# qinhy/Open3D-py-extension

Measured on AMD Instinct MI355X. Metric: Mpoints/sec voxel_down_sample+estimate_normals; ICP iters/sec @ N=10M, higher is better.
Workload: dtype f64

## Files before the change

open3d-py-extension_amd/csrc/grid.hip:

```cpp
#include <type_traits>
#include <utility>

#include "grid.hpp"

namespace o3dx {

__global__ void __launch_bounds__(kBlock) k_grid_count(const float* __restrict__ xyz, int64_t n, GridView g,
                                                       int32_t* __restrict__ count, int32_t* __restrict__ cell,
                                                       int32_t* __restrict__ rank) {
  for (int64_t i = (int64_t)blockIdx.x * blockDim.x + threadIdx.x; i < n; i += (int64_t)gridDim.x * blockDim.x) {
    float x = xyz[3 * i], y = xyz[3 * i + 1], z = xyz[3 * i + 2];
    int cx, cy, cz;
    grid_cell(g, x, y, z, cx, cy, cz);
    const int c = cell_index(g, cx, cy, cz);
    cell[i] = c;
    rank[i] = atomicAdd(&count[c], 1);
  }
}

__global__ void __launch_bounds__(kBlock) k_count_nonzero(const int32_t* __restrict__ count, int64_t nc,
                                                          unsigned long long* __restrict__ out) {
  int64_t local = 0;
  for (int64_t c = (int64_t)blockIdx.x * blockDim.x + threadIdx.x; c < nc; c += (int64_t)gridDim.x * blockDim.x)
    local += count[c] != 0;
// ... 1828 lines not shown
                    wy0 + kVB > d.ny - kEdge || wz0 + kVB > d.nz - kEdge;
  float L = 0.f, U = 0.f;
  int ns = 0, nc = 0;
  if (!fb) {
    if (wide)
      fb = !stile_count_list<Stencil245>(txy, tz, qs, SY, SZ, xpos, q, kneed, d.hlo2, d.rw2, hw, lst, lane, kListMax,
                                         dbg, d, &ns, &nc, &L, &U);
    else
      fb = !stile_count_list<Stencil220>(txy, tz, qs, SY, SZ, xpos, q, kneed, d.hlo2, d.rc2, hw, lst, lane, kListMax,
                                         dbg, d, &ns, &nc, &L, &U);
  }
  if (dbg == 2 || dbg == 3) {
    if (ns + nc == 12345 || L == 12345.f) out[0] = 0.f;
    return;
  }
  if (!fb) {
    const bool over = ns + nc > kListMax;
    if (over && d.stats) atomicAdd(&d.stats[5], 1ull);
    fb = over ||
         !stile_finish<KMAX>(
             q, kneed, ns, nc, L, U, lst, lane,
             [&](int p) { return make_float4(txy[p].x, txy[p].y, tz[p], 0.f); }, prior, oi, out, d.nbr,
             [&](int p) {
               const int bz_ = p / kSZ, r = p - bz_ * kSZ, by_ = r / kSY, bx_ = r - by_ * kSY;
               return __float_as_int(
                   d.vox[(gx0 + bx_) + (int64_t)d.nx * ((gy0 + by_) + (int64_t)d.ny * (gz0 + bz_))].w);
             },
             d.kd2, dbg == 4);
  }
  if (fb) {
    if (d.stats) atomicAdd(&d.stats[4], 1ull);
    const int at = atomicAdd(fb_len, 1);
    fb_list[at] = (int32_t)vq;
  }
}

constexpr int kWaveBnd = 64;
constexpr int kWaveRefineAt = 32;
constexpr int kWavesPerBlock = 4;
constexpr int kWaveCache = 512;

__device__ __forceinline__ void wave_sync() {
  __builtin_amdgcn_fence(__ATOMIC_RELEASE, "wavefront");
  __builtin_amdgcn_wave_barrier();
  __builtin_amdgcn_fence(__ATOMIC_ACQUIRE, "wavefront");
}

__device__ __forceinline__ int lanes_below(uint64_t mask) {
  return (int)__builtin_amdgcn_mbcnt_hi((uint32_t)(mask >> 32), __builtin_amdgcn_mbcnt_lo((uint32_t)mask, 0u));
}

constexpr int kWaveMaxS = 5;
constexpr int kWaveRows = 128;

__device__ __forceinline__ int wave_rows(const GridView& g, const float4 q, int cx, int cy, int cz, int S, float r2,
                                         int lane, int32_t* __restrict__ ra, int32_t* __restrict__ rp) {
  const int side = 2 * S + 1, nr = side * side;
  int carry = 0;
  if (lane == 0) rp[0] = 0;
  for (int h = 0; h * 64 < nr; ++h) {
    const int row = lane + 64 * h;
    int a = 0, len = 0;
    if (row < nr) {
      const int z = cz + row / side - S, y = cy + row % side - S;
      if (z >= 0 && z < g.nz && y >= 0 && y < g.ny) {
        const float y0 = g.oy + (float)y * g.h, z0 = g.oz + (float)z * g.h, sl = 2.0f * g.slack;
        const float dy = fmaxf(fmaxf(y0 - q.y, q.y - (y0 + g.h)) - sl, 0.0f);
        const float dz = fmaxf(fmaxf(z0 - q.z, q.z - (z0 + g.h)) - sl, 0.0f);
        const float rem = r2 - fmaf(dy, dy, dz * dz);
        if (rem > 0.0f) {
          const float rx = sqrtf(rem) + sl;
          const int x0 = max(max(cx - S, 0), (int)floorf((q.x - rx - g.ox) * g.inv_h));
          const int x1 = min(min(cx + S, g.nx - 1), (int)floorf((q.x + rx - g.ox) * g.inv_h));
          if (x0 <= x1) {
            const int rb = g.nx * (y + g.ny * z);
            a = cell_start(g, rb + x0);
            len = cell_start(g, rb + x1 + 1) - a;
          }
        }
      }
    }
    const int inc = wave_incl_scan(len) + carry;
    if (row < nr) {
      ra[row] = a;
      rp[row + 1] = inc;
    }
    carry = __shfl(inc, 63, 64);
  }
  wave_sync();
  return carry;
}

#define O3DX_WAVE_SCAN(S, BODY)                                                  \
  {                                                                              \
    int row_ = 0;                                                                \
    for (int b_ = 0; b_ < ncand; b_ += 64 * WU) {                                \
      float4 v_[WU];                                                             \
      int p_[WU];                                                                \
      _Pragma("unroll") for (int u_ = 0; u_ < WU; ++u_) {                        \
        const int f_ = b_ + u_ * 64 + lane;                                      \
        p_[u_] = -1;                                                             \
        if (f_ < ncand) {                                                        \
          while (rp[row_ + 1] <= f_) ++row_;                                     \
          p_[u_] = ra[row_] + (f_ - rp[row_]);                                   \
        }                                                                        \
        v_[u_] = g.pts[p_[u_] >= 0 ? p_[u_] : 0];                                \
      }                                                                          \
      _Pragma("unroll") for (int u_ = 0; u_ < WU; ++u_) {                        \
        const int pp = p_[u_];                                                   \
        const bool valid = pp >= 0;                                              \
        const int fidx = b_ + u_ * 64 + lane;                                    \
        const float d2 = dist2_f32(q, v_[u_].x, v_[u_].y, v_[u_].z);             \
        (void)fidx;                                                              \
        BODY                                                                     \
      }                                                                          \
    }                                                                            \
  }

#define O3DX_WAVE_SCAN_L(BODY)                                                   \
  for (int b_ = 0; b_ < ncand; b_ += 64) {                                       \
    const int f_ = b_ + lane;                                                    \
    const bool valid = f_ < ncand;                                               \
    const float d2 = valid ? cd2[f_] : 0.0f;                                     \
    const int pp = valid ? cpos[f_] : -1;                                        \
    (void)pp;                                                                    \
    BODY                                                                         \
  }
#define O3DX_WAVE_ANY(BODY)        \
  if (cached) {                    \
    O3DX_WAVE_SCAN_L(BODY)         \
  } else {                         \
    O3DX_WAVE_SCAN(S, BODY)        \
  }

struct Deferred {
  double* mom = nullptr;
  int32_t* row = nullptr;
  int64_t cap = 0;
};

__global__ void __launch_bounds__(kBlock) k_finish_deferred(Deferred df, const int32_t* __restrict__ len, int kneed,
                                                            const float* __restrict__ prior, float* __restrict__ out) {
  const int64_t m = min((int64_t)*len, df.cap);
  for (int64_t t = (int64_t)blockIdx.x * blockDim.x + threadIdx.x; t < m; t += (int64_t)gridDim.x * blockDim.x) {
    const int row = df.row[t];
    if (row < 0) continue;
    MomAcc acc;
#pragma unroll
    for (int j = 0; j < 9; ++j) acc.m[j] = df.mom[j * df.cap + t];
    finish_normal(kneed, acc, prior, row, out);
  }
}

template <int KMAX, int WU>
__device__ __forceinline__ void wave_query(const GridView& g, int kneed, const float* __restrict__ prior,
                                           float* __restrict__ out, int64_t s, int lane, int32_t* sel, int32_t* bnd,
                                           int32_t* __restrict__ ra, int32_t* __restrict__ rp,
                                           float* __restrict__ cd2, int32_t* __restrict__ cpos,
                                           int32_t* __restrict__ fb_list, int32_t* __restrict__ fb_len, int s0,
                                           const Deferred& df, int64_t t) {
  const float4 q = g.pts[s];
  int cx, cy, cz;
  grid_cell(g, q.x, q.y, q.z, cx, cy, cz);
  const int rmax = shell_rmax(g, cx, cy, cz);
  bool fb = false;
  int S = s0;
  float R2 = 0.f;
  RegHist<false> hist;
  int ncand = 0;
  bool cached = false;
  bool trial = s0 == 2;
  float Rd = INFINITY;
  {
    const int c = cell_index(g, cx, cy, cz);
    const int cown = cell_start(g, c + 1) - cell_start(g, c);
    if (cown >= 4 * kneed) Rd = g.h * sqrtf(2.0f * (float)kneed / (float)cown);
  }
  bool dtry = Rd < INFINITY;
  for (;;) {
    if (S >= rmax || S > kWaveMaxS) {
      fb = true;
      break;
    }
    double R = cube_reach(g, q.x, q.y, q.z, cx, cy, cz, S) - g.slack;
    if (trial) R = fmin(R, cube_reach(g, q.x, q.y, q.z, cx, cy, cz, S - 1) - g.slack + 0.5 * (double)g.h);
    if (dtry) R = fmin(R, (double)Rd);
    if (R <= 0.0) {
      ++S;
      trial = false;
      dtry = false;
      continue;
    }
    R2 = (float)(R * R) * (1.0f - 4.0f * kRelEps);
    wave_sync();
    ncand = wave_rows(g, q, cx, cy, cz, S, R2, lane, ra, rp);
    cached = ncand <= kWaveCache;
    const float scale = (float)kHistBins / R2;
    hist.zero();
    int tot = 0;
    O3DX_WAVE_SCAN(S, {
      if (cached && valid) {
        cd2[fidx] = d2;
        cpos[fidx] = pp;
      }
      if (valid && d2 < R2) {
        hist.add(min((int)(d2 * scale), kHistBins - 1));
        ++tot;
      }
    })
    tot = wave_sum(tot);
    if (tot > hist.kMaxTotal) {
      fb = true;
      break;
    }
    if (tot >= kneed) break;
    if (dtry)
      dtry = false;
    else if (trial)
      trial = false;
    else
      ++S;
  }
  wave_sync();
  float lo = 0.f, hi = R2, L = 0.f, U = 0.f;
  int below = 0;
  for (int lvl = 0; !fb; ++lvl) {
#pragma unroll
    for (int i = 0; i < hist.kWords; ++i) hist.h[i] = wave_sum(hist.h[i]);
    int cum, cb;
    if (!hist_locate(hist, kneed, below, lo, hi, &L, &U, &cum, &cb)) {
      fb = true;
      break;
    }
    if (cb <= kWaveRefineAt || lvl == kMaxRefine || !(U > L)) break;
    below += cum;
    lo = L;
    hi = U;
    const float sc = (float)kHistBins / (hi - lo);
    hist.zero();
    O3DX_WAVE_ANY(if (valid && d2 >= lo && d2 < hi) hist.add(min((int)((d2 - lo) * sc), kHistBins - 1));)
  }
  int nsel = 0, nb = 0;
  if (!fb) {
    const float Lm = L * (1.0f - 2.0f * kRelEps), Up = U * (1.0f + 2.0f * kRelEps);
    int nU = 0;
    O3DX_WAVE_ANY({
      nU += __popcll(__ballot(valid && d2 < U));
      const bool c1 = valid && d2 < Lm;
      const bool c2 = valid && !(d2 < Lm) && d2 < Up;
      const uint64_t m1 = __ballot(c1);
      const uint64_t m2 = __ballot(c2);
      if (c1) {
        const int at = nsel + lanes_below(m1);
        if (at < KMAX) sel[at] = pp;
      }
      if (c2) {
        const int at = nb + lanes_below(m2);
        if (at < kWaveBnd) bnd[at] = pp;
      }
      nsel += __popcll(m1);
      nb += __popcll(m2);
    })
    fb = nsel > kneed || nb > kWaveBnd || nsel + nb < kneed || nU < kneed;
  }
  if (!fb) {
    wave_sync();
    const int need = kneed - nsel;
    const double qx = q.x, qy = q.y, qz = q.z;
    double bd = INFINITY;
    int bid = 0x7fffffff, bpos = -1;
    if (lane < nb) {
      bpos = bnd[lane];
      const float4 v = g.pts[bpos];
      bd = dist2_f64(qx, qy, qz, v);
      bid = __float_as_int(v.w);
    }
    int rank = 0;
    for (int i = 0; i < nb; ++i) {
      const double di = __shfl(bd, i, 64);
      const int ii = __shfl(bid, i, 64);
      rank += (di < bd || (di == bd && ii < bid)) ? 1 : 0;
    }
    double cd = -1.0;
    int cid = -1;
    if (lane < nsel) {
      const float4 v = g.pts[sel[lane]];
      cd = dist2_f64(qx, qy, qz, v);
      cid = __float_as_int(v.w);
    }
#pragma unroll
    for (int o = 32; o > 0; o >>= 1) {
      const double od = __shfl_xor(cd, o, 64);
      const int oid = __shfl_xor(cid, o, 64);
      if (od > cd || (od == cd && oid > cid)) {
        cd = od;
        cid = oid;
      }
    }
    if (need < nb && nsel > 0) {
      const uint64_t mk = __ballot(lane < nb && rank == need);
      const int l = __ffsll((unsigned long long)mk) - 1;
      const double ud = __shfl(bd, l, 64);
      const int uid = __shfl(bid, l, 64);
      fb = !(cd < ud || (cd == ud && cid < uid));
    }
    if (!fb) {
      if (lane < nb && rank < need) sel[nsel + rank] = bpos;
      wave_sync();
      double x = 0.0, y = 0.0, z = 0.0;
      if (lane < kneed) {
        const float4 v = g.pts[sel[lane]];
        x = v.x;
        y = v.y;
        z = v.z;
        if (g.nbr) g.nbr[(int64_t)__float_as_int(q.w) * kneed + lane] = __float_as_int(v.w);
      }
      if (g.kd2) {
        double dk = lane < kneed ? dist2_f64(q.x, q.y, q.z, g.pts[sel[lane]]) : 0.0;
#pragma unroll
        for (int o = 32; o > 0; o >>= 1) dk = fmax(dk, __shfl_xor(dk, o, 64));
        if (lane == 0) g.kd2[__float_as_int(q.w)] = (float)(dk * (1.0 + 1e-6));
      }
      MomAcc acc;
      const double t9[9] = {x, y, z, x * x, x * y, x * z, y * y, y * z, z * z};
#pragma unroll
      for (int j = 0; j < 9; ++j) acc.m[j] = wave_sum_exact(t9[j]);
      if (lane == 0) {
        if (t < df.cap) {
#pragma unroll
          for (int j = 0; j < 9; ++j) df.mom[j * df.cap + t] = acc.m[j];
          df.row[t] = __float_as_int(q.w);
        } else {
          finish_normal(kneed, acc, prior, __float_as_int(q.w), out);
        }
      }
    }
  }
  wave_sync();
  if (fb && lane == 0) {
    if (t < df.cap) df.row[t] = -1;
    if (g.stats) atomicAdd(&g.stats[5], 1ull);
    const int at = atomicAdd(fb_len, 1);
    fb_list[at] = (int32_t)s;
  }
}
#undef O3DX_WAVE_SCAN
#undef O3DX_WAVE_SCAN_L
#undef O3DX_WAVE_ANY

template <int KMAX, int WU = 4>
__global__ void __launch_bounds__(64 * kWavesPerBlock) __attribute__((amdgpu_waves_per_eu(4))) k_normals_knn_wave(
    GridView g, int kneed, const float* __restrict__ prior, float* __restrict__ out,
    const int32_t* __restrict__ in_list, const int32_t* __restrict__ in_len, int32_t* __restrict__ fb_list,
    int32_t* __restrict__ fb_len, int s0, Deferred df) {
  __shared__ int32_t sel[kWavesPerBlock][KMAX];
  __shared__ int32_t bnd[kWavesPerBlock][kWaveBnd];
  __shared__ int32_t ra[kWavesPerBlock][kWaveRows];
  __shared__ int32_t rp[kWavesPerBlock][kWaveRows + 1];
  __shared__ float cd2[kWavesPerBlock][kWaveCache];
  __shared__ int32_t cpos[kWavesPerBlock][kWaveCache];
  const int wv = threadIdx.x >> 6, lane = threadIdx.x & 63;
  const int64_t lim = in_list ? (int64_t)*in_len : g.n;
  for (int64_t t = (int64_t)blockIdx.x * kWavesPerBlock + wv; t < lim; t += (int64_t)gridDim.x * kWavesPerBlock) {
    const int64_t s = in_list ? (int64_t)__builtin_amdgcn_readfirstlane(in_list[t]) : t;
    wave_query<KMAX, WU>(g, kneed, prior, out, s, lane, sel[wv], bnd[wv], ra[wv], rp[wv], cd2[wv], cpos[wv], fb_list,
                         fb_len, s0, df, t);
  }
}

__global__ void __launch_bounds__(kBlock) k_normals_radius(GridView g, double radius, const float* __restrict__ prior,
                                                           float* __restrict__ out) {
  const int64_t s = (int64_t)blockIdx.x * blockDim.x + threadIdx.x;
  if (s >= g.n) return;
  const float4 q = g.pts[s];
  const int oi = __float_as_int(q.w);
  int cx, cy, cz;
  grid_cell(g, q.x, q.y, q.z, cx, cy, cz);
  const int rmax = shell_rmax(g, cx, cy, cz);
  const double r2 = radius * radius, qx = q.x, qy = q.y, qz = q.z;
  MomAccDD acc;
  acc.zero();
  int cnt = 0;
  for (int r = 0; r <= rmax; ++r) {
    for_shell(g, cx, cy, cz, r, [&](int c) {
      const int s1 = g.start[c + 1];
      for (int p = g.start[c]; p < s1; ++p) {
        const float4 v = g.pts[p];
        if (dist2_f64(qx, qy, qz, v) < r2) {
          acc.add((double)v.x, (double)v.y, (double)v.z);
          ++cnt;
        }
      }
    });
    if (cube_reach(g, qx, qy, qz, cx, cy, cz, r) - g.slack >= radius) break;
  }
  finish_normal(cnt, acc, prior, oi, out);
}

template <int K>
__global__ void __launch_bounds__(kBlock) k_knn_query(GridView g, const float* __restrict__ q, int64_t nq, int kneed,
                                                      int hybrid, double radius, int kout,
                                                      int32_t* __restrict__ idx_out, double* __restrict__ d2_out,
                                                      int32_t* __restrict__ cnt_out) {
  const int64_t i = (int64_t)blockIdx.x * blockDim.x + threadIdx.x;
  if (i >= nq) return;
  double bd[K];
  int bi[K];
  const int cnt = knn_search_dev<K>(g, q[3 * i], q[3 * i + 1], q[3 * i + 2], kneed, hybrid != 0, radius, bd, bi);
  cnt_out[i] = cnt;
#pragma unroll
  for (int j = 0; j < K; ++j)
    if (j < kout) {
      idx_out[i * kout + j] = j < cnt ? bi[j] : -1;
      if (d2_out) d2_out[i * kout + j] = j < cnt ? bd[j] : INFINITY;
    }
}

static int pick_k(int k) {
  if (k <= 4) return 4;
  if (k <= 8) return 8;
  if (k <= 16) return 16;
  if (k <= 32) return 32;
  return 64;
}

#define O3DX_DISPATCH_K(kk, KERNEL, ...)                                                          \
  switch (pick_k(kk)) {                                                                           \
    case 4: hipLaunchKernelGGL(KERNEL<4>, __VA_ARGS__); break;                                   \
    case 8: hipLaunchKernelGGL(KERNEL<8>, __VA_ARGS__); break;                                   \
    case 16: hipLaunchKernelGGL(KERNEL<16>, __VA_ARGS__); break;                                 \
    case 32: hipLaunchKernelGGL(KERNEL<32>, __VA_ARGS__); break;                                 \
    default: hipLaunchKernelGGL(KERNEL<64>, __VA_ARGS__); break;                                 \
  }

static double occ_for(int mode, int k) {
  if (mode == O3DX_SEARCH_RADIUS) return 4.0;
  if (mode == O3DX_SEARCH_KNN) return std::max(4.0, k / 3.0);
  return std::max(2.0, k / 4.0);
}

template <int B>
__global__ void __launch_bounds__(kBlock) k_vgrid_count(const float4* __restrict__ vox, int vnx, int vny, int vnz,
                                                        GridView g, int32_t* __restrict__ count) {
  const int64_t nc = (int64_t)g.nx * g.ny * g.nz;
  for (int64_t c = (int64_t)blockIdx.x * blockDim.x + threadIdx.x; c < nc; c += (int64_t)gridDim.x * blockDim.x) {
    const int cx = (int)(c % g.nx), cy = (int)((c / g.nx) % g.ny), cz = (int)(c / ((int64_t)g.nx * g.ny));
    int k = 0;
    for (int dz = 0; dz < B; ++dz)
      for (int dy = 0; dy < B; ++dy)
#pragma unroll
        for (int dx = 0; dx < B; ++dx) {
          const int x = cx * B + dx, y = cy * B + dy, z = cz * B + dz;
          if (x < vnx && y < vny && z < vnz)
            k += __float_as_int(vox[x + (int64_t)vnx * (y + (int64_t)vny * z)].w) >= 0;
        }
    count[c] = k;
  }
}

template <int B>
__global__ void __launch_bounds__(kBlock) k_vgrid_emit(const float4* __restrict__ vox, int vnx, int vny, int vnz,
                                                       GridView g, float4* __restrict__ pts) {
  const int64_t nc = (int64_t)g.nx * g.ny * g.nz;
  for (int64_t c = (int64_t)blockIdx.x * blockDim.x + threadIdx.x; c < nc; c += (int64_t)gridDim.x * blockDim.x) {
    const int cx = (int)(c % g.nx), cy = (int)((c / g.nx) % g.ny), cz = (int)(c / ((int64_t)g.nx * g.ny));
    int p = g.start[c];
    for (int dz = 0; dz < B; ++dz)
      for (int dy = 0; dy < B; ++dy)
#pragma unroll
        for (int dx = 0; dx < B; ++dx) {
          const int x = cx * B + dx, y = cy * B + dy, z = cz * B + dz;
          if (x >= vnx || y >= vny || z >= vnz) continue;
          const float4 v = vox[x + (int64_t)vnx * (y + (int64_t)vny * z)];
          if (__float_as_int(v.w) >= 0) pts[p++] = v;
        }
  }
}

static int grid_from_voxels(const double* geom, const float4* vox, int64_t n, double target_occ, void* ws,
                            size_t ws_bytes, hipStream_t s, GridBuild* out) {
  if (!vox || geom[7] != 1.0) return 1;
  const int vn[3] = {(int)geom[4], (int)geom[5], (int)geom[6]};
  const double vs = geom[3];
  GridLayout L = grid_layout(n, 4);
  if (ws_bytes < L.total) return fail(O3DX_ENOMEM, "grid workspace too small (need %zu)", L.total);
  const double occ2 = geom[8];
  if (!(occ2 > 0.0)) return 1;
  const double D = std::min(3.0, std::max(1.0, std::log2((double)n / occ2)));
  int b = 0;
  double best = 0.0;
  for (int c = 1; c <= 4; ++c) {
    int64_t cells = 1;
    for (int a = 0; a < 3; ++a) cells *= (vn[a] + c - 1) / c;
    if (cells > cap_cells(n, 4)) continue;
    const double err = std::fabs(D * std::log((double)c) - std::log(target_occ));
    if (b == 0 || err < best) {
      b = c;
      best = err;
    }
  }
  if (b == 0) return 1;
  char* w = (char*)ws;
  GridBuild& G = *out;
  G.pts = (float4*)(w + L.pts);
  G.start = (int32_t*)(w + L.start);
  G.count = (int32_t*)(w + L.count);
  G.cell = (int32_t*)(w + L.cell);
  G.rank = (int32_t*)(w + L.rank);
  G.scan_tmp = (int32_t*)(w + L.scan);
  G.aabb_ws = w + L.aabb;
  G.mm = (double*)(w + L.mm);
  G.scratch = (int64_t*)(w + L.scratch);
  G.cap_cells = cap_cells(n, 4);
  G.extra = nullptr;
  GridView& g = G.view;
  const double h = b * vs;
  double maxabs = 0.0, maxext = 0.0;
  for (int a = 0; a < 3; ++a) {
    const double ext = vn[a] * vs;
    maxabs = std::max(maxabs, std::max(std::fabs(geom[a]), std::fabs(geom[a] + ext)));
// ... 25 lines not shown
    O3DX_TRY(exclusive_scan_i32(G.count, G.start, nc, G.scan_tmp, s));                                          \
    hipLaunchKernelGGL(k_vgrid_emit<BB>, dim3(gc), dim3(kBlock), 0, s, vox, vn[0], vn[1], vn[2], g, G.pts);      \
    break;
    O3DX_VGRID(1)
    O3DX_VGRID(2)
    O3DX_VGRID(3)
    O3DX_VGRID(4)
#undef O3DX_VGRID
  }
  O3DX_HIP(hipGetLastError());
  return 0;
}

struct SideStream {
  hipStream_t s = nullptr;
  hipEvent_t fork = nullptr, a_done = nullptr, join = nullptr;
};
static SideStream* side_stream(hipStream_t s) {
  constexpr int kMaxDev = 64;
  static thread_local SideStream tab[kMaxDev];
  int cur = -1;
  hipDevice_t sd = -1;
  if (hipGetDevice(&cur) != hipSuccess || hipStreamGetDevice(s, &sd) != hipSuccess || sd != cur || cur < 0 ||
      cur >= kMaxDev)
    return nullptr;
  SideStream& x = tab[cur];
  if (!x.s) {
    SideStream y;
    if (hipStreamCreateWithFlags(&y.s, hipStreamNonBlocking) != hipSuccess) return nullptr;
    if (hipEventCreateWithFlags(&y.fork, hipEventDisableTiming) != hipSuccess ||
        hipEventCreateWithFlags(&y.a_done, hipEventDisableTiming) != hipSuccess ||
        hipEventCreateWithFlags(&y.join, hipEventDisableTiming) != hipSuccess) {
      for (hipEvent_t e : {y.fork, y.a_done, y.join})
        if (e) (void)hipEventDestroy(e);
      (void)hipStreamDestroy(y.s);
      return nullptr;
    }
    x = y;
  }
  return &x;
}

static bool dense_vox_applicable(const double* geom, const float4* vox, int64_t n, int mode, int knn, double* kth) {
  if (!vox || geom[7] != 1.0 || mode != O3DX_SEARCH_KNN || getenv("O3DX_NO_STILE")) return false;
  const int kneed = (int)std::min<int64_t>(knn, n);
  if (kneed < 1 || kneed > 32) return false;
  if (geom[8] == -1.0) {
    *kth = std::cbrt((double)kneed / 4.18879020478639098);
    return true;
  }
  if (!(geom[8] > 0.0)) return false;
  const double dens = (double)n / (8.0 * geom[8]);
  *kth = std::cbrt((double)kneed / (std::min(dens, 1.0) * 4.18879020478639098));
  return dens >= 0.7 && *kth <= 2.0;
}

static int normals_dense_vox(const double* geom, const float4* vox, const float* xyz, int64_t n, int mode, int knn,
                             const float* prior, float* out, float* kd2, void* ws, size_t ws_bytes, hipStream_t s,
                             bool spec = false, bool lens_zeroed = false) {
  double kth = 0.0;
  int kneed = knn;
  if (spec) {
    if (!vox || mode != O3DX_SEARCH_KNN || knn < 1 || knn > 32 || n < knn || getenv("O3DX_NO_STILE")) return 1;
    kth = std::cbrt((double)knn / 4.18879020478639098);
  } else {
    if (!dense_vox_applicable(geom, vox, n, mode, knn, &kth)) return 1;
    kneed = (int)std::min<int64_t>(knn, n);
  }
  DenseVox d;
  d.vox = vox;
  d.nx = (int)geom[4];
  d.ny = (int)geom[5];
  d.nz = (int)geom[6];
  constexpr int wy = 2, wz = 2;
  d.nbx = (d.nx + kVB - 1) / kVB;
  d.nby = (d.ny + kVB * wy - 1) / (kVB * wy);
  d.nbz = (d.nz + kVB * wz - 1) / (kVB * wz);
  const int64_t nb = (int64_t)d.nbx * d.nby * d.nbz;
  if (nb <= 0 || nb > INT32_MAX || (int64_t)d.nx * d.ny * d.nz > INT32_MAX) return 1;
  d.ox = (float)geom[0];
  d.oy = (float)geom[1];
  d.oz = (float)geom[2];
  d.vs = (float)geom[3];
  d.inv_vs = (float)(1.0 / geom[3]);
  double maxabs = 0.0, maxext = 0.0;
  const int vn[3] = {d.nx, d.ny, d.nz};
  for (int a = 0; a < 3; ++a) {
    const double ext = vn[a] * geom[3];
    maxabs = std::max(maxabs, std::max(std::fabs(geom[a]), std::fabs(geom[a] + ext)));
    maxext = std::max(maxext, ext);
  }
  const double slack = 32.0 * std::ldexp(1.0, -24) * (maxabs + maxext) + 1e-6 * geom[3];
  const double R = kStencilR * geom[3] - slack, Rl = kListR * geom[3] - slack;
  d.rc2 = (float)(R * R) * (1.0f - 4.0f * kRelEps);
  d.rl2 = (float)(Rl * Rl) * (1.0f - 4.0f * kRelEps);
  const double Rw = kWideR * geom[3] - slack;
  d.rw2 = (float)(Rw * Rw) * (1.0f - 4.0f * kRelEps);
  d.hlo2 = (float)(kHistLo * geom[3] * kHistLo * geom[3]);
  d.stats = search_stats_ptr();
  d.nbr = debug_nbr(kneed, n);
  d.kd2 = kd2;
  Arena ar((char*)ws, ws_bytes);
  int32_t* lens = ar.take<int32_t>(4);
  int32_t* list = ar.take<int32_t>(n);
  int32_t* list2 = ar.take<int32_t>(n);
  O3DX_ARENA_CHECK(ar);
  if (!lens_zeroed) O3DX_HIP(hipMemsetAsync(lens, 0, 4 * sizeof(int32_t), s));
  const int64_t nint = (int64_t)std::max(d.nbx - 2, 0) * std::max(d.nby - 2, 0) * std::max(d.nbz - 2, 0);
  SideStream* side = nullptr;
  int32_t *list3 = nullptr, *list4 = nullptr;
  const char* want = getenv("O3DX_STILE_SPLIT");
  if (d.nbx >= 3 && d.nby >= 3 && d.nbz >= 3 && want && want[0] == '1') {
    list3 = ar.take<int32_t>(n);
    list4 = ar.take<int32_t>(n);
    if (ar.ok()) side = side_stream(s);
  }
  {
    KTimer kt("normals_knn", s);
    const char* dbg = getenv("O3DX_TILE_DEBUG");
    const int ffb = getenv("O3DX_STILE_FORCE_FB") ? 1 : 0, dg = dbg ? atoi(dbg) : 0;
    KTimer kt_tile("normals_stile", s);
    if (side) {
      O3DX_HIP(hipEventRecord(side->fork, s));
      O3DX_HIP(hipStreamWaitEvent(side->s, side->fork, 0));
      hipLaunchKernelGGL((k_normals_stile<32, wy, wz, 3>), dim3((unsigned)(nb - nint)), dim3(64 * wy * wz), 0,
                         side->s, d, kneed, prior, out, list, lens, ffb, dg, 1);
      O3DX_HIP(hipEventRecord(side->a_done, side->s));
      hipLaunchKernelGGL((k_normals_stile<32, wy, wz, 3>), dim3((unsigned)nint), dim3(64 * wy * wz), 0, s, d, kneed,
                         prior, out, list3, lens + 2, ffb, dg, 2);
      O3DX_HIP(hipStreamWaitEvent(s, side->a_done, 0));
    } else {
      hipLaunchKernelGGL((k_normals_stile<32, wy, wz, 3>), dim3((unsigned)nb), dim3(64 * wy * wz), 0, s, d, kneed,
                         prior, out, list, lens, ffb, dg, 0);
    }
    kt_tile.stop();
    GridView g{};
    g.pts = vox;
    g.start = nullptr;
    g.dense = 1;
    g.ox = (float)geom[0];
    g.oy = (float)geom[1];
    g.oz = (float)geom[2];
    g.h = (float)geom[3];
    g.inv_h = (float)(1.0 / geom[3]);
    g.slack = (float)slack;
    g.nx = d.nx;
    g.ny = d.ny;
    g.nz = d.nz;
    g.n = (int64_t)d.nx * d.ny * d.nz;
    g.stats = d.stats;
    g.nbr = d.nbr;
    g.kd2 = d.kd2;
    auto tail = [&](hipStream_t st, int32_t* l1, int32_t* n1, int32_t* l2, int32_t* n2) {
      hipLaunchKernelGGL(k_normals_knn_wave<32>, dim3(2048), dim3(64 * kWavesPerBlock), 0, st, g, kneed, prior, out,
                         l1, n1, l2, n2, 3, Deferred{});
      hipLaunchKernelGGL(k_normals_knn<32>, dim3(64), dim3(kBlock), 0, st, g, xyz, kneed, 0, 0.0, prior, out, l2,
                         n2);
    };
    if (side) {
      tail(side->s, list, lens, list2, lens + 1);
      O3DX_HIP(hipEventRecord(side->join, side->s));
      KTimer kt_wave("normals_wave", s);
      tail(s, list3, lens + 2, list4, lens + 3);
      kt_wave.stop();
      O3DX_HIP(hipStreamWaitEvent(s, side->join, 0));
    } else {
      KTimer kt_wave("normals_wave", s);
      tail(s, list, lens, list2, lens + 1);
    }
  }
  O3DX_HIP(hipGetLastError());
  return 0;
}

constexpr int64_t kNestedMinQueries = 4096;

template <class F>
__device__ __forceinline__ bool any_around(const GridView& g, int64_t c, F&& f) {
  const int cx = (int)(c % g.nx), cy = (int)((c / g.nx) % g.ny), cz = (int)(c / ((int64_t)g.nx * g.ny));
  for (int z = max(cz - 1, 0); z <= min(cz + 1, g.nz - 1); ++z)
    for (int y = max(cy - 1, 0); y <= min(cy + 1, g.ny - 1); ++y)
      for (int x = max(cx - 1, 0); x <= min(cx + 1, g.nx - 1); ++x)
        if (f((int64_t)x + (int64_t)g.nx * (y + (int64_t)g.ny * z))) return true;
  return false;
}

__global__ void __launch_bounds__(kBlock) k_dense_points(GridView g, int t, unsigned long long* __restrict__ tot) {
  const int64_t nc = (int64_t)g.nx * g.ny * g.nz;
  unsigned long long b = 0;
  for (int64_t c = (int64_t)blockIdx.x * blockDim.x + threadIdx.x; c < nc; c += (int64_t)gridDim.x * blockDim.x) {
    const int own = g.start[c + 1] - g.start[c];
    b += own >= t ? (unsigned long long)own : 0ull;
  }
  b = wave_sum(b);
  if (lane_id() == 0 && b) atomicAdd(tot, b);
}

__global__ void __launch_bounds__(kBlock) k_nested_mark(GridView g, int t, uint8_t* __restrict__ d1) {
  const int64_t nc = (int64_t)g.nx * g.ny * g.nz;
  for (int64_t c = (int64_t)blockIdx.x * blockDim.x + threadIdx.x; c < nc; c += (int64_t)gridDim.x * blockDim.x)
    d1[c] = any_around(g, c, [&](int64_t o) { return g.start[o + 1] - g.start[o] >= t; }) ? 1 : 0;
}

__global__ void __launch_bounds__(kBlock) k_nested_cells(GridView g, const uint8_t* __restrict__ d1,
                                                         int32_t* __restrict__ sub_cnt,
                                                         unsigned long long* __restrict__ tot) {
  const int64_t nc = (int64_t)g.nx * g.ny * g.nz;
  unsigned long long a = 0, b = 0;
  for (int64_t c = (int64_t)blockIdx.x * blockDim.x + threadIdx.x; c < nc; c += (int64_t)gridDim.x * blockDim.x) {
    const int own = g.start[c + 1] - g.start[c];
    const bool d2 = own > 0 && any_around(g, c, [&](int64_t o) { return d1[o] != 0; });
    sub_cnt[c] = d2 ? own : 0;
    a += d2 ? (unsigned long long)own : 0ull;
    b += d1[c] ? (unsigned long long)own : 0ull;
  }
  a = wave_sum(a);
  b = wave_sum(b);
  if (lane_id() == 0 && (a | b)) {
    atomicAdd(&tot[0], a);
    atomicAdd(&tot[1], b);
  }
}

__global__ void __launch_bounds__(kBlock) k_nested_gather(GridView g, const uint8_t* __restrict__ d1,
                                                          const int32_t* __restrict__ sub_cnt,
                                                          const int32_t* __restrict__ sub_off,
                                                          float* __restrict__ sub_xyz, int32_t* __restrict__ sub_id) {
  for (int64_t p = (int64_t)blockIdx.x * blockDim.x + threadIdx.x; p < g.n; p += (int64_t)gridDim.x * blockDim.x) {
    const float4 v = g.pts[p];
    int cx, cy, cz;
    grid_cell(g, v.x, v.y, v.z, cx, cy, cz);
    const int c = cell_index(g, cx, cy, cz);
    if (sub_cnt[c] == 0) continue;
    const int64_t d = (int64_t)sub_off[c] + (p - g.start[c]);
    sub_xyz[3 * d] = v.x;
    sub_xyz[3 * d + 1] = v.y;
    sub_xyz[3 * d + 2] = v.z;
    sub_id[d] = d1[c] ? (int32_t)p : -(int32_t)p - 1;
  }
}

struct NestedWs {
  int32_t *sub_cnt, *sub_off, *scan_tmp, *chunks;
  uint8_t* d1;
  unsigned long long* tot;
  float* sub_xyz;
  int32_t* sub_id;
  void *gws, *pws;
  size_t gws_bytes, pws_bytes;
  int64_t cap;
};

static void nested_carve(Arena& ar, int64_t n, NestedWs& w) {
  const int64_t nc = cap_cells(std::max<int64_t>(n, 1), 4);
  w.cap = n / 2 + 4096;
  w.d1 = ar.take<uint8_t>(nc + 1);
  w.sub_cnt = ar.take<int32_t>(nc + 1);
  w.sub_off = ar.take<int32_t>(nc + 1);
  w.scan_tmp = ar.take<int32_t>(scan_workspace_ints(nc + 1));
  w.tot = ar.take<unsigned long long>(3);
  w.sub_xyz = ar.take<float>(3 * w.cap);
  w.sub_id = ar.take<int32_t>(w.cap);
  w.gws_bytes = grid_ws_bytes(w.cap);
  w.gws = ar.take<char>(w.gws_bytes);
  const int64_t rows = cap_cells(w.cap, 4);
  w.chunks = ar.take<int32_t>(w.cap / kTileQ + rows + 4);
  w.pws_bytes = chunk_plan_ws_bytes(w.cap, rows);
  w.pws = ar.take<char>(w.pws_bytes);
}

static size_t nested_ws_bytes(int64_t n) {
  Arena ar(nullptr, 0);
  NestedWs w;
  nested_carve(ar, n, w);
  return ar.used;
}

static int nested_tiles(GridBuild& G, int64_t n, int kneed, double occ, const float* prior, float* out,
                        int32_t* fb_list, int32_t* fb_len, Arena& ar, hipStream_t s) {
  NestedWs w;
  nested_carve(ar, n, w);
  O3DX_ARENA_CHECK(ar);
  const int t = (int)std::ceil(4.0 * occ);
  const int64_t nc = (int64_t)G.view.nx * G.view.ny * G.view.nz;
  KTimer kt("normals_nested", s);
  O3DX_HIP(hipMemsetAsync(w.tot, 0, 3 * sizeof(unsigned long long), s));
  const unsigned gc = grid_for(nc, kBlock, 4096);
  hipLaunchKernelGGL(k_dense_points, dim3(gc), dim3(kBlock), 0, s, G.view, t, w.tot + 2);
  unsigned long long dense = 0;
  O3DX_TRY(read_back(&dense, w.tot + 2, sizeof(dense), s));
  const int64_t minq = std::max<int64_t>(kNestedMinQueries, n / 32);
  if ((int64_t)dense < minq) return 0;
  hipLaunchKernelGGL(k_nested_mark, dim3(gc), dim3(kBlock), 0, s, G.view, t, w.d1);
  hipLaunchKernelGGL(k_nested_cells, dim3(gc), dim3(kBlock), 0, s, G.view, w.d1, w.sub_cnt, w.tot);
  unsigned long long tot[2];
  O3DX_TRY(read_back(tot, w.tot, sizeof(tot), s));
  const int64_t nsub = (int64_t)tot[0];
  if (nsub > w.cap) return 0;
  O3DX_TRY(exclusive_scan_i32(w.sub_cnt, w.sub_off, nc, w.scan_tmp, s));
  hipLaunchKernelGGL(k_nested_gather, dim3(grid_for(n, kBlock, 8192)), dim3(kBlock), 0, s, G.view, w.d1, w.sub_cnt,
                     w.sub_off, w.sub_xyz, w.sub_id);
  GridBuild N;
  O3DX_TRY(grid_build(w.sub_xyz, nsub, occ, 0.0, w.gws, w.gws_bytes, s, &N, nullptr, nullptr, false, 4, false,
                      w.sub_id, 0.5 * (double)G.view.h));
  GridView& v = N.view;
  v.outer = G.view.pts;
  v.cox = G.view.ox;
  v.coy = G.view.oy;
// ... 738 lines not shown
```

Before: 13460.

## Add dense-voxel handoff kNN kernel with per-lane precomputed cube offsets

Adds a specialised wave kernel for the dense voxel grid's handoff list. Each lane holds precomputed neighbor-cell offset codes for the 7^3 cube and the radius-4 shell, so each voxel is loaded directly with no cell-range scans. It counts against the reach radius, refines with the shared histogram locator, and finishes with the exact f64 selection, which is factored into reusable helpers. This removes the generic shell iteration and LDS caching in the wave kernel, at the cost of more registers per lane and a different occupancy hint.

```diff
diff --git a/open3d-py-extension_amd/csrc/grid.hip b/open3d-py-extension_amd/csrc/grid.hip
--- a/open3d-py-extension_amd/csrc/grid.hip
+++ b/open3d-py-extension_amd/csrc/grid.hip
@@ -2004,6 +2004,147 @@
   }
 }
 
+template <class Rebin>
+__device__ __forceinline__ bool wave_locate(RegHist<false>& hist, int kneed, float R2, float* L, float* U,
+                                            Rebin&& rebin) {
+  float lo = 0.f, hi = R2;
+  int below = 0;
+  for (int lvl = 0;; ++lvl) {
+#pragma unroll
+    for (int i = 0; i < hist.kWords; ++i) hist.h[i] = wave_sum(hist.h[i]);
+    int cum, cb;
+    if (!hist_locate(hist, kneed, below, lo, hi, L, U, &cum, &cb)) return false;
+    if (cb <= kWaveRefineAt || lvl == kMaxRefine || !(*U > *L)) return true;
+    below += cum;
+    lo = *L;
+    hi = *U;
+    const float sc = (float)kHistBins / (hi - lo);
+    hist.zero();
+    rebin(lo, hi, sc);
+  }
+}
+
+template <int KMAX>
+struct WaveLists {
+  int32_t* sel;
+  int32_t* bnd;
+  int nsel = 0, nb = 0, nU = 0;
+  float Lm = 0.f, U = 0.f, Up = 0.f;
+  __device__ __forceinline__ void bounds(float L, float U_) {
+    Lm = L * (1.0f - 2.0f * kRelEps);
+    U = U_;
+    Up = U_ * (1.0f + 2.0f * kRelEps);
+  }
+  __device__ __forceinline__ void add(bool valid, float d2, int pp) {
+    nU += __popcll(__ballot(valid && d2 < U));
+    const bool c1 = valid && d2 < Lm;
+    const bool c2 = valid && !(d2 < Lm) && d2 < Up;
+    const uint64_t m1 = __ballot(c1);
+    const uint64_t m2 = __ballot(c2);
+    if (c1) {
+      const int at = nsel + lanes_below(m1);
+      if (at < KMAX) sel[at] = pp;
+    }
+    if (c2) {
+      const int at = nb + lanes_below(m2);
+      if (at < kWaveBnd) bnd[at] = pp;
+    }
+    nsel += __popcll(m1);
+    nb += __popcll(m2);
+  }
+  __device__ __forceinline__ bool ok(int kneed) const {
+    return !(nsel > kneed || nb > kWaveBnd || nsel + nb < kneed || nU < kneed);
+  }
+};
+
+__device__ __forceinline__ bool wave_finish_exact(const GridView& g, const float4 q, int kneed, int nsel, int nb,
+                                                  int32_t* sel, int32_t* bnd, int lane,
+                                                  const float* __restrict__ prior, float* __restrict__ out,
+                                                  const Deferred& df, int64_t t) {
+  wave_sync();
+  const int need = kneed - nsel;
+  const double qx = q.x, qy = q.y, qz = q.z;
+  double bd = INFINITY;
+  int bid = 0x7fffffff, bpos = -1;
+  if (lane < nb) {
+    bpos = bnd[lane];
+    const float4 v = g.pts[bpos];
+    bd = dist2_f64(qx, qy, qz, v);
+    bid = __float_as_int(v.w);
+  }
+  int rank = 0;
+  for (int i = 0; i < nb; ++i) {
+    const double di = __shfl(bd, i, 64);
+    const int ii = __shfl(bid, i, 64);
+    rank += (di < bd || (di == bd && ii < bid)) ? 1 : 0;
+  }
+  double cd = -1.0;
+  int cid = -1;
+  if (lane < nsel) {
+    const float4 v = g.pts[sel[lane]];
+    cd = dist2_f64(qx, qy, qz, v);
+    cid = __float_as_int(v.w);
+  }
+#pragma unroll
+  for (int o = 32; o > 0; o >>= 1) {
+    const double od = __shfl_xor(cd, o, 64);
+    const int oid = __shfl_xor(cid, o, 64);
+    if (od > cd || (od == cd && oid > cid)) {
+      cd = od;
+      cid = oid;
+    }
+  }
+  if (need < nb && nsel > 0) {
+    const uint64_t mk = __ballot(lane < nb && rank == need);
+    const int l = __ffsll((unsigned long long)mk) - 1;
+    const double ud = __shfl(bd, l, 64);
+    const int uid = __shfl(bid, l, 64);
+    if (!(cd < ud || (cd == ud && cid < uid))) return false;
+  }
+  if (lane < nb && rank < need) sel[nsel + rank] = bpos;
+  wave_sync();
+  double x = 0.0, y = 0.0, z = 0.0;
+  if (lane < kneed) {
+    const float4 v = g.pts[sel[lane]];
+    x = v.x;
+    y = v.y;
+    z = v.z;
+    if (g.nbr) g.nbr[(int64_t)__float_as_int(q.w) * kneed + lane] = __float_as_int(v.w);
+  }
+  if (g.kd2) {
+    double dk = lane < kneed ? dist2_f64(q.x, q.y, q.z, g.pts[sel[lane]]) : 0.0;
+#pragma unroll
+    for (int o = 32; o > 0; o >>= 1) dk = fmax(dk, __shfl_xor(dk, o, 64));
+    if (lane == 0) g.kd2[__float_as_int(q.w)] = (float)(dk * (1.0 + 1e-6));
+  }
+  MomAcc acc;
+  const double t9[9] = {x, y, z, x * x, x * y, x * z, y * y, y * z, z * z};
+#pragma unroll
+  for (int j = 0; j < 9; ++j) acc.m[j] = wave_sum_exact(t9[j]);
+  if (lane == 0) {
+    if (t < df.cap) {
+#pragma unroll
+      for (int j = 0; j < 9; ++j) df.mom[j * df.cap + t] = acc.m[j];
+      df.row[t] = __float_as_int(q.w);
+    } else {
+      finish_normal(kneed, acc, prior, __float_as_int(q.w), out);
+    }
+  }
+  return true;
+}
+
+__device__ __forceinline__ void wave_pass_on(const GridView& g, bool fb, int64_t s, int lane,
+                                             int32_t* __restrict__ fb_list, int32_t* __restrict__ fb_len,
+                                             const Deferred& df, int64_t t) {
+  wave_sync();
+  if (fb && lane == 0) {
+    if (t < df.cap) df.row[t] = -1;
+    if (g.stats) atomicAdd(&g.stats[5], 1ull);
+    const int at = atomicAdd(fb_len, 1);
+    fb_list[at] = (int32_t)s;
+  }
+}
+
 template <int KMAX, int WU>
 __device__ __forceinline__ void wave_query(const GridView& g, int kneed, const float* __restrict__ prior,
                                            float* __restrict__ out, int64_t s, int lane, int32_t* sel, int32_t* bnd,
@@ -2074,127 +2215,19 @@
       ++S;
   }
   wave_sync();
-  float lo = 0.f, hi = R2, L = 0.f, U = 0.f;
-  int below = 0;
-  for (int lvl = 0; !fb; ++lvl) {
-#pragma unroll
-    for (int i = 0; i < hist.kWords; ++i) hist.h[i] = wave_sum(hist.h[i]);
-    int cum, cb;
-    if (!hist_locate(hist, kneed, below, lo, hi, &L, &U, &cum, &cb)) {
-      fb = true;
-      break;
-    }
-    if (cb <= kWaveRefineAt || lvl == kMaxRefine || !(U > L)) break;
-    below += cum;
-    lo = L;
-    hi = U;
-    const float sc = (float)kHistBins / (hi - lo);
-    hist.zero();
-    O3DX_WAVE_ANY(if (valid && d2 >= lo && d2 < hi) hist.add(min((int)((d2 - lo) * sc), kHistBins - 1));)
-  }
-  int nsel = 0, nb = 0;
+  float L = 0.f, U = 0.f;
+  if (!fb)
+    fb = !wave_locate(hist, kneed, R2, &L, &U, [&](float lo, float hi, float sc) {
+      O3DX_WAVE_ANY(if (valid && d2 >= lo && d2 < hi) hist.add(min((int)((d2 - lo) * sc), kHistBins - 1));)
+    });
+  WaveLists<KMAX> wl{sel, bnd};
   if (!fb) {
-    const float Lm = L * (1.0f - 2.0f * kRelEps), Up = U * (1.0f + 2.0f * kRelEps);
-    int nU = 0;
-    O3DX_WAVE_ANY({
-      nU += __popcll(__ballot(valid && d2 < U));
-      const bool c1 = valid && d2 < Lm;
-      const bool c2 = valid && !(d2 < Lm) && d2 < Up;
-      const uint64_t m1 = __ballot(c1);
-      const uint64_t m2 = __ballot(c2);
-      if (c1) {
-        const int at = nsel + lanes_below(m1);
-        if (at < KMAX) sel[at] = pp;
-      }
-      if (c2) {
-        const int at = nb + lanes_below(m2);
-        if (at < kWaveBnd) bnd[at] = pp;
-      }
-      nsel += __popcll(m1);
-      nb += __popcll(m2);
-    })
-    fb = nsel > kneed || nb > kWaveBnd || nsel + nb < kneed || nU < kneed;
-  }
-  if (!fb) {
-    wave_sync();
-    const int need = kneed - nsel;
-    const double qx = q.x, qy = q.y, qz = q.z;
-    double bd = INFINITY;
-    int bid = 0x7fffffff, bpos = -1;
-    if (lane < nb) {
-      bpos = bnd[lane];
-      const float4 v = g.pts[bpos];
-      bd = dist2_f64(qx, qy, qz, v);
-      bid = __float_as_int(v.w);
-    }
-    int rank = 0;
-    for (int i = 0; i < nb; ++i) {
-      const double di = __shfl(bd, i, 64);
-      const int ii = __shfl(bid, i, 64);
-      rank += (di < bd || (di == bd && ii < bid)) ? 1 : 0;
-    }
-    double cd = -1.0;
-    int cid = -1;
-    if (lane < nsel) {
-      const float4 v = g.pts[sel[lane]];
-      cd = dist2_f64(qx, qy, qz, v);
-      cid = __float_as_int(v.w);
-    }
-#pragma unroll
-    for (int o = 32; o > 0; o >>= 1) {
-      const double od = __shfl_xor(cd, o, 64);
-      const int oid = __shfl_xor(cid, o, 64);
-      if (od > cd || (od == cd && oid > cid)) {
-        cd = od;
-        cid = oid;
-      }
-    }
-    if (need < nb && nsel > 0) {
-      const uint64_t mk = __ballot(lane < nb && rank == need);
-      const int l = __ffsll((unsigned long long)mk) - 1;
-      const double ud = __shfl(bd, l, 64);
-      const int uid = __shfl(bid, l, 64);
-      fb = !(cd < ud || (cd == ud && cid < uid));
-    }
-    if (!fb) {
-      if (lane < nb && rank < need) sel[nsel + rank] = bpos;
-      wave_sync();
-      double x = 0.0, y = 0.0, z = 0.0;
-      if (lane < kneed) {
-        const float4 v = g.pts[sel[lane]];
-        x = v.x;
-        y = v.y;
-        z = v.z;
-        if (g.nbr) g.nbr[(int64_t)__float_as_int(q.w) * kneed + lane] = __float_as_int(v.w);
-      }
-      if (g.kd2) {
-        double dk = lane < kneed ? dist2_f64(q.x, q.y, q.z, g.pts[sel[lane]]) : 0.0;
-#pragma unroll
-        for (int o = 32; o > 0; o >>= 1) dk = fmax(dk, __shfl_xor(dk, o, 64));
-        if (lane == 0) g.kd2[__float_as_int(q.w)] = (float)(dk * (1.0 + 1e-6));
-      }
-      MomAcc acc;
-      const double t9[9] = {x, y, z, x * x, x * y, x * z, y * y, y * z, z * z};
-#pragma unroll
-      for (int j = 0; j < 9; ++j) acc.m[j] = wave_sum_exact(t9[j]);
-      if (lane == 0) {
-        if (t < df.cap) {
-#pragma unroll
-          for (int j = 0; j < 9; ++j) df.mom[j * df.cap + t] = acc.m[j];
-          df.row[t] = __float_as_int(q.w);
-        } else {
-          finish_normal(kneed, acc, prior, __float_as_int(q.w), out);
-        }
-      }
-    }
-  }
-  wave_sync();
-  if (fb && lane == 0) {
-    if (t < df.cap) df.row[t] = -1;
-    if (g.stats) atomicAdd(&g.stats[5], 1ull);
-    const int at = atomicAdd(fb_len, 1);
-    fb_list[at] = (int32_t)s;
-  }
+    wl.bounds(L, U);
+    O3DX_WAVE_ANY(wl.add(valid, d2, pp);)
+    fb = !wl.ok(kneed);
+  }
+  if (!fb) fb = !wave_finish_exact(g, q, kneed, wl.nsel, wl.nb, sel, bnd, lane, prior, out, df, t);
+  wave_pass_on(g, fb, s, lane, fb_list, fb_len, df, t);
 }
 #undef O3DX_WAVE_SCAN
 #undef O3DX_WAVE_SCAN_L
@@ -2218,6 +2251,144 @@
     wave_query<KMAX, WU>(g, kneed, prior, out, s, lane, sel[wv], bnd[wv], ra[wv], rp[wv], cd2[wv], cpos[wv], fb_list,
                          fb_len, s0, df, t);
   }
+}
+
+constexpr int kVoxN3 = 6;
+constexpr int kVoxN4 = 7;
+constexpr int kVoxNC = kVoxN3 + kVoxN4;
+
+__device__ __forceinline__ int vox_code(int dx, int dy, int dz) { return (dx + 4) | ((dy + 4) << 4) | ((dz + 4) << 8); }
+__device__ __forceinline__ int vox_cube3_code(int i) {
+  const int r = i % 49;
+  return i < 343 ? vox_code(r % 7 - 3, r / 7 - 3, i / 49 - 3) : -1;
+}
+
+__device__ __forceinline__ int vox_shell4_code(int i) {
+  if (i >= 386) return -1;
+  if (i < 162) {
+    const int r = i % 81;
+    return vox_code(r % 9 - 4, r / 9 - 4, i < 81 ? -4 : 4);
+  }
+  const int t = i - 162, r = t % 32, dz = t / 32 - 3;
+  if (r < 18) return vox_code(r % 9 - 4, r < 9 ? -4 : 4, dz);
+  return vox_code(((r - 18) & 1) ? 4 : -4, ((r - 18) >> 1) - 3, dz);
+}
+
+__device__ __forceinline__ int vox_slot(const GridView& g, int cx, int cy, int cz, int code) {
+  const int x = cx + (code & 15) - 4, y = cy + ((code >> 4) & 15) - 4, z = cz + ((code >> 8) & 15) - 4;
+  const bool ok = code >= 0 && x >= 0 && x < g.nx && y >= 0 && y < g.ny && z >= 0 && z < g.nz;
+  return ok ? x + g.nx * (y + g.ny * z) : -1;
+}
+
+template <int B, int N>
+__device__ __forceinline__ void vox_load_cells(const GridView& g, const float4 q, int cx, int cy, int cz,
+                                               const int (&code)[kVoxNC], float (&d2)[kVoxNC]) {
+  float4 v[N];
+#pragma unroll
+  for (int j = 0; j < N; ++j) {
+    const int p = vox_slot(g, cx, cy, cz, code[B + j]);
+    v[j] = make_float4(0.f, 0.f, 0.f, __int_as_float(-1));
+    if (p >= 0) v[j] = g.pts[p];
+  }
+#pragma unroll
+  for (int j = 0; j < N; ++j) {
+    const float d = dist2_f32(q, v[j].x, v[j].y, v[j].z);
+    d2[B + j] = (__float_as_int(v[j].w) >= 0 && d < INFINITY) ? d : INFINITY;
+  }
+}
+
+template <int NC>
+__device__ __forceinline__ int vox_count(const float (&d2)[kVoxNC], float R2, RegHist<false>& hist) {
+  const float scale = (float)kHistBins / R2;
+  hist.zero();
+  int tot = 0;
+#pragma unroll
+  for (int j = 0; j < NC; ++j)
+    if (d2[j] < R2) {
+      hist.add(min((int)(d2[j] * scale), kHistBins - 1));
+      ++tot;
+    }
+  return wave_sum(tot);
+}
+
+template <int KMAX>
+__device__ __forceinline__ bool vox_select(const GridView& g, const float4 q, int cx, int cy, int cz, int kneed,
+                                           float R2, RegHist<false>& hist, const int (&code)[kVoxNC],
+                                           const float (&d2)[kVoxNC], int32_t* sel, int32_t* bnd, int lane,
+                                           const float* __restrict__ prior, float* __restrict__ out) {
+  float L = 0.f, U = 0.f;
+  if (!wave_locate(hist, kneed, R2, &L, &U, [&](float lo, float hi, float sc) {
+#pragma unroll
+        for (int j = 0; j < kVoxNC; ++j)
+          if (d2[j] >= lo && d2[j] < hi) hist.add(min((int)((d2[j] - lo) * sc), kHistBins - 1));
+      }))
+    return false;
+  WaveLists<KMAX> wl{sel, bnd};
+  wl.bounds(L, U);
+#pragma unroll
+  for (int j = 0; j < kVoxNC; ++j) wl.add(true, d2[j], vox_slot(g, cx, cy, cz, code[j]));
+  if (!wl.ok(kneed)) return false;
+  return wave_finish_exact(g, q, kneed, wl.nsel, wl.nb, sel, bnd, lane, prior, out, Deferred{}, 0);
+}
+
+__device__ __forceinline__ float vox_reach2(const GridView& g, const float4 q, int cx, int cy, int cz, int S) {
+  const double R = cube_reach(g, q.x, q.y, q.z, cx, cy, cz, S) - g.slack;
+  return R > 0.0 ? (float)(R * R) * (1.0f - 4.0f * kRelEps) : 0.0f;
+}
+
+template <int KMAX>
+__device__ __forceinline__ void vox_handoff_query(const GridView& g, int kneed, const float* __restrict__ prior,
+                                                  float* __restrict__ out, const int32_t* __restrict__ in_list,
+                                                  int64_t t, int (&code)[kVoxNC], int32_t* sel, int32_t* bnd,
+                                                  int lane, int32_t* __restrict__ fb_list,
+                                                  int32_t* __restrict__ fb_len) {
+#pragma unroll
+  for (int j = 0; j < kVoxNC; ++j) asm volatile("" : "+v"(code[j]));
+  const int s = __builtin_amdgcn_readfirstlane(in_list[t]);
+  const float4 q = g.pts[s];
+  const int cx = s % g.nx, cy = (s / g.nx) % g.ny, cz = s / (g.nx * g.ny);
+  const int rmax = shell_rmax(g, cx, cy, cz);
+  float d2[kVoxNC];
+  RegHist<false> hist;
+  float R2 = 0.f;
+  bool fb = 3 >= rmax;
+  if (!fb) {
+    vox_load_cells<0, kVoxN3>(g, q, cx, cy, cz, code, d2);
+    R2 = vox_reach2(g, q, cx, cy, cz, 3);
+    if (vox_count<kVoxN3>(d2, R2, hist) >= kneed) {
+#pragma unroll
+      for (int j = kVoxN3; j < kVoxNC; ++j) d2[j] = INFINITY;
+    } else if (4 >= rmax) {
+      fb = true;
+    } else {
+      vox_load_cells<kVoxN3, kVoxN4>(g, q, cx, cy, cz, code, d2);
+      R2 = vox_reach2(g, q, cx, cy, cz, 4);
+      fb = vox_count<kVoxNC>(d2, R2, hist) < kneed;
+    }
+  }
+  if (!fb) fb = !vox_select<KMAX>(g, q, cx, cy, cz, kneed, R2, hist, code, d2, sel, bnd, lane, prior, out);
+  wave_pass_on(g, fb, s, lane, fb_list, fb_len, Deferred{}, t);
+}
+
+template <int KMAX>
+__global__ void __launch_bounds__(64 * kWavesPerBlock) __attribute__((amdgpu_waves_per_eu(6, 6)))
+k_normals_vox_handoff(GridView g, int kneed, const float* __restrict__ prior, float* __restrict__ out,
+                      const int32_t* __restrict__ in_list, const int32_t* __restrict__ in_len,
+                      int32_t* __restrict__ fb_list, int32_t* __restrict__ fb_len) {
+  __shared__ int32_t sel[kWavesPerBlock][KMAX];
+  __shared__ int32_t bnd[kWavesPerBlock][kWaveBnd];
+  const int wv = threadIdx.x >> 6, lane = threadIdx.x & 63;
+  const int64_t lim = *in_len, stride = (int64_t)gridDim.x * kWavesPerBlock;
+  int64_t t = (int64_t)blockIdx.x * kWavesPerBlock + wv;
+  if (t >= lim) return;
+  int code[kVoxNC];
+#pragma unroll
+  for (int j = 0; j < kVoxN3; ++j) code[j] = vox_cube3_code(lane + 64 * j);
+#pragma unroll
+  for (int j = 0; j < kVoxN4; ++j) code[kVoxN3 + j] = vox_shell4_code(lane + 64 * j);
+  vox_handoff_query<KMAX>(g, kneed, prior, out, in_list, t, code, sel[wv], bnd[wv], lane, fb_list, fb_len);
+  for (t += stride; t < lim; t += stride)
+    vox_handoff_query<KMAX>(g, kneed, prior, out, in_list, t, code, sel[wv], bnd[wv], lane, fb_list, fb_len);
 }
 
 __global__ void __launch_bounds__(kBlock) k_normals_radius(GridView g, double radius, const float* __restrict__ prior,
@@ -2549,8 +2720,8 @@
     g.nbr = d.nbr;
     g.kd2 = d.kd2;
     auto tail = [&](hipStream_t st, int32_t* l1, int32_t* n1, int32_t* l2, int32_t* n2) {
-      hipLaunchKernelGGL(k_normals_knn_wave<32>, dim3(2048), dim3(64 * kWavesPerBlock), 0, st, g, kneed, prior, out,
-                         l1, n1, l2, n2, 3, Deferred{});
+      hipLaunchKernelGGL(k_normals_vox_handoff<32>, dim3(2048), dim3(64 * kWavesPerBlock), 0, st, g, kneed, prior,
+                         out, l1, n1, l2, n2);
       hipLaunchKernelGGL(k_normals_knn<32>, dim3(64), dim3(kBlock), 0, st, g, xyz, kneed, 0, 0.0, prior, out, l2,
                          n2);
     };
```

Result: no change. 13580 (median of 6 runs) (+0.9%).
